# AleixMT/TrigenicInteractionPredictor

Measured on NVIDIA B200. Metric: EM link-updates/sec at K=10, higher is better.
Workload: dtype f64

## Files before the change

### include/tip.h

```cpp
#ifndef TIP_H_
#define TIP_H_

#include <stddef.h>
#include <stdint.h>

#ifdef __cplusplus
extern "C" {
#endif

#define TIP_ABI_VERSION 1
#define TIP_EPS 1e-10
#define TIP_R 2
#define TIP_MAX_K 32

#define TIP_EM_DEFAULT 0u
#define TIP_EM_FORCE_GENERIC 1u
#define TIP_EM_FP32_COMPUTE 2u
#define TIP_EM_GENE_SEGMENTED 8u
#define TIP_EM_SLOT_SEGMENTED 32u
#define TIP_EM_GATHER_L1 64u
#define TIP_EM_WITH_LOGLIK 4u

#define TIP_ROWS_COMPACT8 16u

// ... 13 lines not shown
int tip_order_rows_by_gene(const void *d_rows, int64_t n_rows, int64_t n_rows_r0, int P, void *d_ws, size_t ws_bytes,
                           void *d_rows_bc, void *stream);
int tip_order_rows(const void *d_rows, int64_t n_rows, int64_t n_rows_r0, void *d_ws, size_t ws_bytes, void *d_rows_bc,
                   void *stream);

int tip_em_workspace_bytes(int P, int K, int64_t n_rows, unsigned flags, size_t *bytes);
int tip_em_step(int P, int K, const void *d_rows, int64_t n_rows, int64_t n_rows_r0, const double *d_theta,
                const double *d_p, double *d_stats, void *d_ws, size_t ws_bytes, unsigned flags, void *stream);

int tip_em_step_host_rows(int P, int K, const void *h_rows, int64_t n_rows, int64_t n_rows_r0, unsigned row_flags,
                          void *d_rows_dev, const double *d_theta, const double *d_p, double *d_stats, void *d_ws,
                          size_t ws_bytes, unsigned *d_err, void *stream, void *copy_stream);

int tip_normalise(int P, int K, const double *d_stats, const int32_t *d_deg, double *d_theta, double *d_p,
                  void *stream);

size_t tip_loglik_workspace_bytes(int P, int K);
int tip_loglik(int P, int K, const void *d_rows, int64_t n_rows, int64_t n_rows_r0, const double *d_theta,
               const double *d_p, double *d_out, void *d_ws, unsigned flags, void *stream);

int tip_score(int P, int K, const int32_t *d_g1, const int32_t *d_g2, const int32_t *d_g3, int64_t T,
              const double *d_theta, const double *d_p, double *d_scores, void *stream);

int tip_metrics_workspace_bytes(int64_t T, size_t *bytes);
int tip_metrics(const double *d_scores, const int32_t *d_labels, int64_t T, int64_t positives_number,
                void *d_ws, size_t ws_bytes, int64_t *d_out, void *stream);

int tip_sort_scores_workspace_bytes(int64_t T, size_t *bytes);
int tip_sort_scores(const double *d_scores, int64_t T, void *d_ws, size_t ws_bytes, int32_t *d_order, double *d_sorted,
                    void *stream);
// ... 47 lines not shown
```

### trigenicinteractionpredictor_b200/_cabi.py

```python
from __future__ import annotations

import ctypes
import os
import re

HERE = os.path.dirname(os.path.abspath(__file__))
LIB_PATH = os.path.join(HERE, "libtip.so")
HEADER = os.path.join(os.path.dirname(HERE), "include", "tip.h")

c_void_p, c_int, c_int64, c_size_t, c_uint, c_double = (
    ctypes.c_void_p, ctypes.c_int, ctypes.c_int64, ctypes.c_size_t, ctypes.c_uint, ctypes.c_double)
_pi64 = ctypes.POINTER(ctypes.c_int64)
_psz = ctypes.POINTER(ctypes.c_size_t)
_pdbl = ctypes.POINTER(ctypes.c_double)

TIP_EM_DEFAULT = 0
TIP_EM_FORCE_GENERIC = 1
TIP_EM_FP32_COMPUTE = 2
TIP_EM_WITH_LOGLIK = 4
TIP_EM_GENE_SEGMENTED = 8
TIP_ROWS_COMPACT8 = 16
TIP_EM_SLOT_SEGMENTED = 32
TIP_EM_GATHER_L1 = 64

# ... 3 lines not shown
    "tip_stats_len": (c_int64, [c_int, c_int]),
    "tip_rows_capacity": (c_int64, [c_int64]),
    "tip_pack_rows_workspace_bytes": (c_int, [c_int64, _psz]),
    "tip_pack_rows": (c_int, [c_void_p, c_void_p, c_void_p, c_void_p, c_void_p, c_int64, c_int, c_void_p, c_size_t,
                              c_void_p, _pi64, _pi64, c_void_p, c_void_p]),
    "tip_order_rows_workspace_bytes": (c_int, [c_int64, _psz]),
    "tip_order_rows_out_bytes": (c_int64, [c_int64]),
    "tip_order_rows_by_gene": (c_int, [c_void_p, c_int64, c_int64, c_int, c_void_p, c_size_t, c_void_p, c_void_p]),
    "tip_order_rows": (c_int, [c_void_p, c_int64, c_int64, c_void_p, c_size_t, c_void_p, c_void_p]),
    "tip_em_workspace_bytes": (c_int, [c_int, c_int, c_int64, c_uint, _psz]),
    "tip_em_step": (c_int, [c_int, c_int, c_void_p, c_int64, c_int64, c_void_p, c_void_p, c_void_p, c_void_p, c_size_t,
                            c_uint, c_void_p]),
    "tip_em_step_host_rows": (c_int, [c_int, c_int, c_void_p, c_int64, c_int64, c_uint, c_void_p, c_void_p, c_void_p, c_void_p,
                                      c_void_p, c_size_t, c_void_p, c_void_p, c_void_p]),
    "tip_normalise": (c_int, [c_int, c_int, c_void_p, c_void_p, c_void_p, c_void_p, c_void_p]),
    "tip_loglik_workspace_bytes": (c_size_t, [c_int, c_int]),
    "tip_loglik": (c_int, [c_int, c_int, c_void_p, c_int64, c_int64, c_void_p, c_void_p, c_void_p, c_void_p, c_uint,
                           c_void_p]),
    "tip_score": (c_int, [c_int, c_int, c_void_p, c_void_p, c_void_p, c_int64, c_void_p, c_void_p, c_void_p, c_void_p]),
    "tip_metrics_workspace_bytes": (c_int, [c_int64, _psz]),
    "tip_metrics": (c_int, [c_void_p, c_void_p, c_int64, c_int64, c_void_p, c_size_t, c_void_p, c_void_p]),
    "tip_sort_scores_workspace_bytes": (c_int, [c_int64, _psz]),
    "tip_sort_scores": (c_int, [c_void_p, c_int64, c_void_p, c_size_t, c_void_p, c_void_p, c_void_p]),
    "tip_top_triplets_workspace_bytes": (c_int, [c_int, c_int, c_int, c_int64, c_int64, _psz]),
    "tip_top_triplets": (c_int, [c_int, c_int, c_int, c_void_p, c_void_p, c_void_p, c_int, c_void_p, c_int64, c_int64, c_void_p,
                                 c_size_t, c_void_p, c_void_p, _pi64, c_void_p]),
    "tip_top_triplets_last_passes": (c_int, []),
    "tip_reduce_samples": (c_int, [c_int, c_int64, c_void_p, c_void_p, c_void_p, c_void_p, c_void_p, c_void_p, c_void_p]),
    "tip_em_iterations_host": (c_int, [c_int, c_int, c_void_p, c_int64, c_int64, c_void_p, c_void_p, c_void_p, c_int,
                                       c_uint]),
# ... 81 lines not shown
```

### trigenicinteractionpredictor_b200/csrc/tip_api.cu

```cuda
#include <stdarg.h>
#include <string.h>

#include <chrono>

#include "tip_common.cuh"

namespace tip {

static thread_local char g_err[512] = "";

void set_error(const char *fmt, ...)
{
    va_list ap;
    va_start(ap, fmt);
    vsnprintf(g_err, sizeof(g_err), fmt, ap);
    va_end(ap);
}

static bool valid_K(int K) { return K >= 1 && K <= TIP_MAX_K; }
static bool uses_tuned(int K, unsigned flags)
{
    if (flags & TIP_EM_FORCE_GENERIC) return false;
    if (K <= 10) return true;
    return !(flags & (TIP_EM_WITH_LOGLIK | TIP_EM_FP32_COMPUTE));
// ... 10 lines not shown

extern "C" int64_t tip_stats_len(int P, int K) { return (int64_t)P * K + 2ll * K * K * K + 1; }

extern "C" int tip_em_workspace_bytes(int P, int K, int64_t n_rows, unsigned flags, size_t *bytes)
{
    TIP_REQUIRE(bytes != nullptr && P > 0 && valid_K(K) && n_rows >= 0, "tip_em_workspace_bytes: bad arguments");
    if (seg3_flag(flags)) {
        *bytes = em_seg3_workspace_bytes(P, K, n_rows);
        return 0;
    }
    *bytes = uses_tuned(K, flags) ? em_tuned_workspace_bytes(P, K, seg_flag(flags))
                                  : (size_t)(n_rows < 1 ? 1 : n_rows) * sizeof(double);
    return 0;
}

extern "C" int tip_em_step(int P, int K, const void *d_rows, int64_t n_rows, int64_t n_rows_r0, const double *d_theta,
                           const double *d_p, double *d_stats, void *d_ws, size_t ws_bytes, unsigned flags, void *stream)
{
    cudaStream_t st = reinterpret_cast<cudaStream_t>(stream);
    TIP_REQUIRE(P > 0 && valid_K(K), "tip_em_step: need P > 0 and 1 <= K <= %d (got P=%d K=%d)", TIP_MAX_K, P, K);
    TIP_REQUIRE(n_rows >= 0 && n_rows % 32 == 0 && n_rows_r0 >= 0 && n_rows_r0 <= n_rows && n_rows_r0 % 32 == 0,
                "tip_em_step: n_rows (%lld) and n_rows_r0 (%lld) must be multiples of 32 from tip_pack_rows",
                (long long)n_rows, (long long)n_rows_r0);
    TIP_REQUIRE(d_theta && d_p && d_stats && (d_rows || n_rows == 0), "tip_em_step: null pointer");
    TIP_REQUIRE(!(flags & TIP_EM_FP32_COMPUTE) || (K <= 10 && !(flags & (TIP_EM_FORCE_GENERIC | TIP_EM_WITH_LOGLIK))),
                "tip_em_step: TIP_EM_FP32_COMPUTE exists for the K <= 10 kernels only, without FORCE_GENERIC / WITH_LOGLIK");
    TIP_REQUIRE(!seg_flag(flags) || !(flags & (TIP_EM_FORCE_GENERIC | TIP_EM_WITH_LOGLIK | TIP_EM_FP32_COMPUTE)),
                "tip_em_step: TIP_EM_GENE_SEGMENTED cannot be combined with other mode flags");
    TIP_REQUIRE(!seg3_flag(flags) || (flags & ~(TIP_EM_SLOT_SEGMENTED | TIP_EM_GATHER_L1)) == 0,
                "tip_em_step: TIP_EM_SLOT_SEGMENTED combines with TIP_EM_GATHER_L1 only");
    TIP_REQUIRE(seg3_flag(flags) || !(flags & TIP_EM_GATHER_L1), "tip_em_step: TIP_EM_GATHER_L1 needs TIP_EM_SLOT_SEGMENTED");
    TIP_CHECK_CUDA(cudaMemsetAsync(d_stats, 0, sizeof(double) * (size_t)tip_stats_len(P, K), st));
    if (n_rows == 0) return 0;
    const int4 *rows = reinterpret_cast<const int4 *>(d_rows);
    if (seg3_flag(flags)) {
        const size_t need = em_seg3_workspace_bytes(P, K, n_rows);
        TIP_REQUIRE(d_ws != nullptr && ws_bytes >= need,
                    "tip_em_step: the slot-segmented mode needs %zu bytes of workspace (got %zu), see tip_em_workspace_bytes",
                    need, ws_bytes);
        return launch_em_seg3(P, K, rows, n_rows, n_rows_r0, d_theta, d_p, d_stats, reinterpret_cast<double *>(d_ws),
                              (flags & TIP_EM_GATHER_L1) != 0, st);
    }
    if (uses_tuned(K, flags)) {
        const size_t need = em_tuned_workspace_bytes(P, K, seg_flag(flags));
        TIP_REQUIRE(need == 0 || (d_ws != nullptr && ws_bytes >= need),
                    "tip_em_step: K=%d needs %zu bytes of workspace (got %zu), see tip_em_workspace_bytes", K, need, ws_bytes);
        bool handled = false;
        int rc = launch_em_tuned(P, K, rows, n_rows, n_rows_r0, d_theta, d_p, d_stats, reinterpret_cast<double *>(d_ws),
                                 (flags & TIP_EM_WITH_LOGLIK) != 0, (flags & TIP_EM_FP32_COMPUTE) != 0, seg_flag(flags), st,
                                 &handled);
        if (rc != 0 || handled) return rc;
    }
    TIP_REQUIRE(d_ws != nullptr && ws_bytes >= (size_t)n_rows * sizeof(double),
                "tip_em_step: the any-K path needs %zu bytes of workspace (got %zu)", (size_t)n_rows * sizeof(double), ws_bytes);
    return launch_em_generic(P, K, rows, n_rows, n_rows_r0, d_theta, d_p, d_stats, reinterpret_cast<double *>(d_ws), st);
}

extern "C" int tip_em_step_host_rows(int P, int K, const void *h_rows, int64_t n_rows, int64_t n_rows_r0, unsigned row_flags,
                                     void *d_rows_dev, const double *d_theta, const double *d_p, double *d_stats, void *d_ws,
                                     size_t ws_bytes, unsigned *d_err, void *stream, void *copy_stream)
{
    cudaStream_t st = reinterpret_cast<cudaStream_t>(stream), cs = reinterpret_cast<cudaStream_t>(copy_stream);
    TIP_REQUIRE(P > 0 && valid_K(K) && em_streamed_available(K, false, false, false),
                "tip_em_step_host_rows: the streamed E-step exists for the plain fp64 K <= 10 kernels (got K=%d); copy the "
                "rows and call tip_em_step", K);
    TIP_REQUIRE(n_rows > 0 && n_rows % 32 == 0 && n_rows_r0 >= 0 && n_rows_r0 <= n_rows && n_rows_r0 % 32 == 0,
                "tip_em_step_host_rows: n_rows (%lld) and n_rows_r0 (%lld) must be multiples of 32 from tip_pack_rows",
                (long long)n_rows, (long long)n_rows_r0);
    TIP_REQUIRE(h_rows && d_rows_dev && d_theta && d_p && d_stats && d_err && cs != st && (row_flags & ~TIP_ROWS_COMPACT8) == 0,
                "tip_em_step_host_rows: bad arguments (two distinct streams are required)");
// ... 172 lines not shown
        return rc;
    if (seg3 && n_iter > 0 && n_rows >= 32 && getenv("TIP_HOST_SEG3_AFTER_STREAM") == nullptr) {
        TIP_CHECK_CUDA(cudaMemcpyAsync(g.theta, h_theta, nth, cudaMemcpyHostToDevice, g.st));
        TIP_CHECK_CUDA(cudaMemcpyAsync(g.p, h_p, np, cudaMemcpyHostToDevice, g.st));
        TIP_CHECK_CUDA(cudaMemcpyAsync(compact ? g.rows8 : g.rows, h_rows, (size_t)n_rows * row_b, cudaMemcpyHostToDevice, g.st));
        if (compact && (rc = launch_rows_expand(g.rows8, g.rows, n_rows, g.st))) return rc;
        TIP_CHECK_CUDA(cudaEventRecord(g.ev_rows, g.st));
        TIP_CHECK_CUDA(cudaMemcpyAsync(g.deg, h_deg, (size_t)P * 4, cudaMemcpyHostToDevice, g.st));
        char *rows_bc = (char *)g.rows + (size_t)n_rows * 16;
        TIP_CHECK_CUDA(cudaStreamWaitEvent(g.copy, g.ev_rows, 0));
        if ((rc = order_rows_parts(g.rows, n_rows, n_rows_r0, g.order_ws2, g.order_ws2_b, rows_bc, g.copy, 2, P))) return rc;
        TIP_CHECK_CUDA(cudaEventRecord(g.ev_ordered, g.copy));
        if ((rc = order_rows_parts(g.rows, n_rows, n_rows_r0, g.order_ws, g.order_ws_b, rows_bc, g.st, 1, P))) return rc;
        for (int it = 0; it < n_iter; ++it) {
            if (it == 0) seg3_wait_before_bc(g.ev_ordered);
            rc = tip_em_step(P, K, g.rows, n_rows, n_rows_r0, (const double *)g.theta, (const double *)g.p, (double *)g.stats,
                             g.ws, g.ws_b, flags, g.st);
            if (rc) return rc;
            rc = launch_normalise(P, K, (const double *)g.stats, (const int32_t *)g.deg, (double *)g.theta, (double *)g.p, g.st);
            if (rc) return rc;
        }
        TIP_CHECK_CUDA(cudaMemcpyAsync(h_theta, g.theta, nth, cudaMemcpyDeviceToHost, g.st));
        TIP_CHECK_CUDA(cudaMemcpyAsync(h_p, g.p, np, cudaMemcpyDeviceToHost, g.st));
        TIP_CHECK_CUDA(cudaStreamSynchronize(g.st));
        return 0;
    }
    const bool tuned = uses_tuned(K, flags & ~(TIP_EM_SLOT_SEGMENTED | TIP_EM_GATHER_L1));
    const bool streamed = tuned && n_iter > 0 && n_rows >= 32 * kHostChunks &&
                          em_streamed_available(K, (flags & TIP_EM_WITH_LOGLIK) != 0, (flags & TIP_EM_FP32_COMPUTE) != 0,
                                                seg_flag(flags)) && getenv("TIP_HOST_NO_STREAM") == nullptr;
    char *s_dst = compact ? (char *)g.rows8 : (char *)g.rows;
    TIP_CHECK_CUDA(cudaMemcpyAsync(g.theta, h_theta, nth, cudaMemcpyHostToDevice, g.st));
    TIP_CHECK_CUDA(cudaMemcpyAsync(g.p, h_p, np, cudaMemcpyHostToDevice, g.st));
    if (!streamed) TIP_CHECK_CUDA(cudaMemcpyAsync(g.deg, h_deg, (size_t)P * 4, cudaMemcpyHostToDevice, g.st));
// ... 288 lines not shown
```

### trigenicinteractionpredictor_b200/csrc/tip_common.cuh

```cuda
#pragma once
#include <cuda_runtime.h>
#include <stdint.h>
#include <stdio.h>

#include "tip.h"

namespace tip {

constexpr int kWarp = 32;
constexpr int kNumSM_B200 = 148;

void set_error(const char *fmt, ...);

#define TIP_CHECK_CUDA(expr)                                                                   \
    do {                                                                                       \
        cudaError_t _e = (expr);                                                               \
        if (_e != cudaSuccess) {                                                               \
            ::tip::set_error("%s failed: %s (%s:%d)", #expr, cudaGetErrorString(_e), __FILE__, \
                             __LINE__);                                                        \
            return -2;                                                                         \
        }                                                                                      \
    } while (0)

#define TIP_REQUIRE(cond, ...)             \
// ... 44 lines not shown
template <int N>
__device__ __forceinline__ void cp_async_wait()
{
    asm volatile("cp.async.wait_group %0;" ::"n"(N) : "memory");
}

__host__ __device__ inline int64_t stats_off_S(int P, int K) { return (int64_t)P * K; }
__host__ __device__ inline int64_t stats_off_ll(int P, int K) { return (int64_t)P * K + 2ll * K * K * K; }

int launch_em_generic(int P, int K, const int4 *rows, int64_t n_rows, int64_t n_rows_r0, const double *theta,
                      const double *p, double *stats, double *s_ws, cudaStream_t st);
int launch_em_tuned(int P, int K, const int4 *rows, int64_t n_rows, int64_t n_rows_r0, const double *theta,
                    const double *p, double *stats, double *ws, bool with_ll, bool f32, bool seg, cudaStream_t st,
                    bool *handled, int phases = 7);
size_t em_tuned_workspace_bytes(int P, int K, bool seg);
int launch_em_seg3(int P, int K, const int4 *rows, int64_t n_rows, int64_t n_rows_r0, const double *theta, const double *p,
                   double *stats, double *ws, bool gather_l1, cudaStream_t st);
size_t em_seg3_workspace_bytes(int P, int K, int64_t n_rows);
int order_rows_parts(const void *d_rows, int64_t n_rows, int64_t n_rows_r0, void *d_ws, size_t ws_bytes, void *d_rows_bc,
                     cudaStream_t st, int parts, int P);
void seg3_wait_before_bc(cudaEvent_t ev);
cudaEvent_t seg3_take_bc_wait();
bool em_streamed_available(int K, bool with_ll, bool f32, bool seg);
int launch_em_streamed(int P, int K, const void *rows, int64_t n_rows, int64_t n_rows_r0, const double *theta, double *stats,
                       double *ws, unsigned *err, unsigned long long *chk, bool compact, cudaStream_t st);
int launch_stream_verify(const void *rows, int64_t n_rows, bool compact, unsigned long long *chk, unsigned *err, cudaStream_t st);
int launch_loglik(int P, int K, const int4 *rows, int64_t n_rows, int64_t n_rows_r0, const double *theta, const double *p,
                  double *out, void *ws, bool force_generic, cudaStream_t st);
int launch_loglik_seg(int P, int K, const int4 *rows, int64_t n_rows, const double *theta, const double *p, double *out,
                      double *partials, unsigned *counter, int max_blocks, double *Zws, cudaStream_t st);
size_t loglik_seg_workspace_bytes(int P, int K);
int launch_loglik_tuned(int K, const int4 *rows, int64_t n_rows, int64_t n_rows_r0, const double *theta, const double *p,
// ... 9 lines not shown
```

### trigenicinteractionpredictor_b200/csrc/tip_seg3.cu

```cuda
#include <stdlib.h>

#include <cub/device/device_radix_sort.cuh>

#include "tip_common.cuh"

namespace tip {

__device__ __forceinline__ void dmma884(double &c0, double &c1, double a, double b)
{
    asm volatile("mma.sync.aligned.m8n8k4.row.col.f64.f64.f64.f64 {%0,%1}, {%2}, {%3}, {%0,%1};"
                 : "+d"(c0), "+d"(c1)
                 : "d"(a), "d"(b));
}

__device__ __forceinline__ void red_add_f64_nz3(double *addr, double v)
{
    asm volatile("{ .reg .pred p; setp.neu.f64 p, %1, 0d0000000000000000; @p red.global.add.f64 [%0], %1; }" ::"l"(addr),
                 "d"(v)
                 : "memory");
}

__device__ __forceinline__ void st_relaxed_gpu_f64(double *addr, double v)
{
    asm volatile("st.relaxed.gpu.global.f64 [%0], %1;" ::"l"(addr), "d"(v) : "memory");
// ... 93 lines not shown
            copy(idw[l * 4 + 1 + slot], l, slot, (rem - slot * C::U) * C::UNIT);
        }
    }
}

template <int K, bool FIRST, int NST, bool CA>
__global__ void __launch_bounds__(32, K <= 16 ? (FIRST ? 16 : 18) : 1) seg3_pass_kernel(const S3Args a)
{
    using C = S3<K>;
    constexpr int KK = C::KK, NB = C::NB, NKG = C::NKG, RS = C::RS, D = NST - 1;
    extern __shared__ __align__(16) unsigned char smem_raw[];
    const int lane = threadIdx.x, li = lane & 3, ri = lane >> 2;
    if constexpr (FIRST) {
        asm volatile("griddepcontrol.wait;" ::: "memory");
        asm volatile("griddepcontrol.launch_dependents;" ::: "memory");
    }
    auto stage_of = [&](int b) { return reinterpret_cast<double *>(smem_raw + (size_t)b * C::BUF_BYTES); };
    auto ids_of = [&](int b) { return reinterpret_cast<int4 *>(stage_of(b) + 32 * RS + 32); };
    int xo[NB];
    bool xv[NB];
#pragma unroll
    for (int i = 0; i < NB; ++i) {
        xv[i] = i * 8 + ri < K;
        xo[i] = xv[i] ? i * 8 + ri : 0;
    }

    double acc[NB][NB][2];
#pragma unroll
    for (int i = 0; i < NB; ++i)
#pragma unroll
// ... 276 lines not shown
        __syncwarp();
#pragma unroll
        for (int j = 0; j + 1 < D + RQ; ++j) tq[j] = tq[j + 1];
        tq[D + RQ - 1] = tn;
        if (++cb == NST) cb = 0;
    }
}

constexpr int kPrepGenes = 16;
__global__ void __launch_bounds__(256) seg3_prep_kernel(int P, int K, const double *__restrict__ theta,
                                                        const double *__restrict__ p, double *__restrict__ Zg,
                                                        double *__restrict__ PT, double *__restrict__ thpad, int TP,
                                                        double2 *__restrict__ zero2, int64_t n_zero2,
                                                        double2 *__restrict__ nan2, int64_t n_nan2,
                                                        unsigned *__restrict__ cnt_a, unsigned cnt_a0,
                                                        unsigned *__restrict__ cnt_bc, unsigned cnt_bc0)
{
    asm volatile("griddepcontrol.launch_dependents;" ::: "memory");
    if (blockIdx.x == 0 && threadIdx.x == 0) {
        *cnt_a = cnt_a0;
        *cnt_bc = cnt_bc0;
    }
    extern __shared__ double psm[];
    const int KK = K * K, K3 = KK * K;
    const bool staged = K <= 20;
    double *tsm = psm + (staged ? 2 * K3 : 0);
    const int g0 = blockIdx.x * kPrepGenes;
    const int ng = (P - g0 < kPrepGenes) ? P - g0 : kPrepGenes;
    constexpr int PB = 8;
    double pv[PB];
    const int e_th = threadIdx.x;
    double tv = 0.0;
    if (e_th < ng * K) tv = __ldg(theta + (int64_t)g0 * K + e_th);
    if (staged) {
#pragma unroll
        for (int j = 0; j < PB; ++j) {
            const int e = threadIdx.x + j * 256;
// ... 54 lines not shown
        else if (slot == 1) { i = x; j = k; l = y; }
        else { i = x; j = y; l = k; }
        PT[f] = __ldg(p + (((int64_t)i * K + j) * K + l) * 2 + r);
    }
}

constexpr int kFin3Threads = 96;
constexpr int kFin3GeneChunk = 96;
constexpr int kS3MaxPeers = 16;

struct S3Push {
    int n;
    double *dst[kS3MaxPeers];
};

template <int K>
__global__ void __launch_bounds__(kFin3Threads) seg3_finish_kernel(int P, const double *__restrict__ theta,
                                                                     const double *__restrict__ PT,
                                                                     const double *__restrict__ Mg, double *__restrict__ stats,
                                                                     const S3Push push)
{
    constexpr int KK = K * K, K3 = KK * K, NB = (K + 7) / 8, NBC = (KK + 7) / 8;
    const int lane = threadIdx.x & 31, li = lane & 3, ri = lane >> 2, warp = threadIdx.x >> 5;
    const int n_groups = (P + 7) / 8;
    const int n_chunks = (P + kFin3GeneChunk - 1) / kFin3GeneChunk, n_kind2 = 2 * NBC * n_chunks;
    __shared__ double csm[2][NB * 2][32];
    if ((int)blockIdx.x < n_groups) {
        const int slot = warp, g = blockIdx.x * 8 + ri;
        const bool gv = g < P;
        double c[NB][2];
#pragma unroll
        for (int i = 0; i < NB; ++i) c[i][0] = c[i][1] = 0.0;
        constexpr int NE = (KK + 3) / 4;
        constexpr int EB = NE < 32 ? NE : 32;
        for (int r = 0; r < 2; ++r) {
            const double *Mrow = Mg + ((int64_t)(slot * 2 + r) * P + (gv ? g : 0)) * KK;
// ... 24 lines not shown
            for (int i = 0; i < NB; ++i) {
                csm[warp - 1][2 * i][lane] = c[i][0];
                csm[warp - 1][2 * i + 1][lane] = c[i][1];
            }
        }
        __syncthreads();
        if (warp == 0) {
            __shared__ __align__(16) double rowbuf[8 * K + 2];
            if (gv) {
#pragma unroll
                for (int i = 0; i < NB; ++i)
#pragma unroll
                    for (int h = 0; h < 2; ++h) {
                        const int k = i * 8 + 2 * li + h;
                        if (k < K)
                            rowbuf[ri * K + k] = __ldg(theta + (int64_t)g * K + k) *
                                                 ((c[i][h] + csm[0][2 * i + h][lane]) + csm[1][2 * i + h][lane]);
                    }
            }
            __syncwarp();
            const int g0 = blockIdx.x * 8, ng = (P - g0 < 8) ? P - g0 : 8, nd = ng * K;
            const int64_t at0 = (int64_t)g0 * K;
            for (int q = -1; q < push.n; ++q) {
                double *dst = (q < 0 ? stats : push.dst[q]) + at0;
                for (int i = lane; i < nd / 2; i += 32) reinterpret_cast<double2 *>(dst)[i] = reinterpret_cast<const double2 *>(rowbuf)[i];
                if ((nd & 1) && lane == 0) dst[nd - 1] = rowbuf[nd - 1];
            }
        }
        return;
    }
    const int wt = ((int)blockIdx.x - n_groups) * (kFin3Threads / 32) + warp;
    if (wt < n_kind2) {
        const int w2 = wt;
        const int chunk = w2 / (2 * NBC), rem = w2 - chunk * (2 * NBC), r = rem / NBC, bcb = rem - r * NBC;
        const int g_lo = chunk * kFin3GeneChunk, g_hi = (g_lo + kFin3GeneChunk < P) ? g_lo + kFin3GeneChunk : P;
        const int bc = bcb * 8 + ri;
        const double *Mr = Mg + (int64_t)r * P * KK;
        double c[NB][2];
#pragma unroll
        for (int i = 0; i < NB; ++i) c[i][0] = c[i][1] = 0.0;
#pragma unroll 4
        for (int g0 = g_lo; g0 < g_hi; g0 += 4) {
            const int g = g0 + li;
            const bool gv = g < g_hi;
            const double bv = (gv && bc < KK) ? __ldg(Mr + (int64_t)g * KK + bc) : 0.0;
#pragma unroll
            for (int i = 0; i < NB; ++i) {
                const int al = i * 8 + ri;
                const double av = (gv && al < K) ? __ldg(theta + (int64_t)g * K + al) : 0.0;
                dmma884(c[i][0], c[i][1], av, bv);
            }
        }
        double *S = stats + stats_off_S(P, K) + (int64_t)r * K3;
#pragma unroll
        for (int i = 0; i < NB; ++i)
#pragma unroll
            for (int h = 0; h < 2; ++h) {
                const int al = i * 8 + ri, cell = bcb * 8 + 2 * li + h;
                if (al < K && cell < KK) red_add_f64_nz3(S + (int64_t)al * KK + cell, c[i][h]);
            }
    }
}

struct S3Layout {
    size_t off_M, off_cnt, off_Z, off_PT, off_T, off_s, total;
};
static S3Layout s3_layout(int P, int K, int64_t n_rows)
{
    const size_t KK = (size_t)K * K;
    S3Layout l;
    l.off_M = 0;
    l.off_cnt = 6 * (size_t)P * KK;
    l.off_Z = l.off_cnt + kS3CounterDoubles;
    l.off_PT = l.off_Z + 2 * (size_t)P * KK;
    l.off_PT = (l.off_PT + 1) / 2 * 2;
// ... 45 lines not shown
    if (!g_s3_ev[0])
        for (int j = 0; j < 6; ++j) TIP_CHECK_CUDA(cudaEventCreate(&g_s3_ev[j]));
    TIP_CHECK_CUDA(cudaEventRecord(g_s3_ev[i], st));
    return 0;
}

static bool s3_no_overlap()
{
    static int v = -1;
    if (v < 0) {
        const char *e = getenv("TIP_SEG3_NO_OVERLAP");
        v = (e && atoi(e) != 0) ? 1 : 0;
    }
    return v != 0;
}

template <int K, bool FIRST, int NST, bool CA>
static int s3_launch_pass_n(const S3Args &a, cudaStream_t st, int *grid_only)
{
    using C = S3<K>;
    constexpr size_t smem = C::BUF_BYTES * NST;
    static int blocks_per_sm = 0;
    if (blocks_per_sm == 0) {
        TIP_CHECK_CUDA(cudaFuncSetAttribute(seg3_pass_kernel<K, FIRST, NST, CA>, cudaFuncAttributeMaxDynamicSharedMemorySize, (int)smem));
        TIP_CHECK_CUDA(cudaFuncSetAttribute(seg3_pass_kernel<K, FIRST, NST, CA>, cudaFuncAttributePreferredSharedMemoryCarveout,
                                            cudaSharedmemCarveoutMaxShared));
        int nb = 0;
        TIP_CHECK_CUDA(cudaOccupancyMaxActiveBlocksPerMultiprocessor(&nb, seg3_pass_kernel<K, FIRST, NST, CA>, 32, smem));
        TIP_REQUIRE(nb >= 1, "seg3_pass_kernel<%d> does not fit on an SM (smem %zu)", K, smem);
        blocks_per_sm = nb;
// ... 25 lines not shown
}

template <int K, bool FIRST>
static int s3_launch_pass(const S3Args &a, cudaStream_t st, int *grid_only = nullptr)
{
    const bool ca = (a.tune & 1) != 0;
    if (s3_stages(FIRST) == 1)
        return ca ? s3_launch_pass_n<K, FIRST, 1, true>(a, st, grid_only) : s3_launch_pass_n<K, FIRST, 1, false>(a, st, grid_only);
    return ca ? s3_launch_pass_n<K, FIRST, 2, true>(a, st, grid_only) : s3_launch_pass_n<K, FIRST, 2, false>(a, st, grid_only);
}

static S3Push g_s3_push = {};

template <int K>
static int launch_em_seg3_k(int P, const int4 *rows, int64_t n_rows, int64_t n_rows_r0, const double *theta, const double *p,
                            double *stats, double *ws, bool gather_l1, cudaStream_t st)
{
    const S3Push push = g_s3_push;
    g_s3_push.n = 0;
    const cudaEvent_t bc_wait = seg3_take_bc_wait();
    const S3Layout l = s3_layout(P, K, n_rows);
    const int KK = K * K;
    TIP_REQUIRE(n_rows / 32 < (1ll << 27), "tip_em_step: too many tiles in one shard for the slot-segmented kernels");
    const int skip = s3_skip();
    S3Args a;
    a.P = P;
    a.rows = rows;
    a.tiles_per_order = (int)(n_rows / 32);
    a.n_tiles_r0 = (int)(n_rows_r0 / 32);
    a.theta = ws + l.off_T;
    a.Zg = ws + l.off_Z;
// ... 6 lines not shown
    const int *sched = reinterpret_cast<const int *>(rows + 3 * n_rows);
    a.sched = sched;
    a.n_sched = a.tiles_per_order;
    S3Args bc = a;
    bc.rows = rows + n_rows;
    bc.n_tiles = 2 * a.tiles_per_order;
    bc.slot0 = 1;
    bc.counter = reinterpret_cast<unsigned *>(ws + l.off_cnt) + kS3Groups * 32;
    bc.sched = sched + a.tiles_per_order;
    bc.n_sched = 2 * a.tiles_per_order;
    int grid_a = 0, grid_bc = 0;
    int rc = s3_launch_pass<K, true>(a, st, &grid_a);
    if (rc) return rc;
    rc = s3_launch_pass<K, false>(bc, st, &grid_bc);
    if (rc) return rc;
    if (s3_mark(0, st)) return -2;
    if (s3_mark(1, st)) return -2;
    {
        const size_t smem = sizeof(double) * ((K <= 20 ? 2 * KK * K : 0) + kPrepGenes * K);
        static bool attr = false;
        if (!attr && smem > 48 * 1024) {
            TIP_CHECK_CUDA(cudaFuncSetAttribute(seg3_prep_kernel, cudaFuncAttributeMaxDynamicSharedMemorySize, 128 * 1024));
            attr = true;
        }
        seg3_prep_kernel<<<(P + kPrepGenes - 1) / kPrepGenes, 256, smem, st>>>(
            P, K, theta, p, ws + l.off_Z, ws + l.off_PT, ws + l.off_T, S3<K>::TP, reinterpret_cast<double2 *>(ws + l.off_M),
            (int64_t)l.off_cnt / 2, reinterpret_cast<double2 *>(ws + l.off_s), (n_rows < 32 ? 32 : n_rows) / 2, a.counter,
            2u * (unsigned)grid_a, bc.counter, 2u * (unsigned)grid_bc);
        TIP_CHECK_CUDA(cudaGetLastError());
    }
    if (s3_mark(2, st)) return -2;
    rc = (skip & 4) ? 0 : s3_launch_pass<K, true>(a, st);
    if (rc) return rc;
    if (s3_mark(3, st)) return -2;
    if (bc_wait) {
        TIP_CHECK_CUDA(cudaStreamWaitEvent(st, bc_wait, 0));
        bc.tune |= 16;
    }
    rc = (skip & 8) ? 0 : s3_launch_pass<K, false>(bc, st);
    if (rc) return rc;
    if (s3_mark(4, st)) return -2;
    if (!(skip & 16)) {
        constexpr int NBC = (K * K + 7) / 8;
        const int n_kind2 = 2 * NBC * ((P + kFin3GeneChunk - 1) / kFin3GeneChunk);
        const int wpc = kFin3Threads / 32;
        seg3_finish_kernel<K><<<(P + 7) / 8 + (n_kind2 + wpc - 1) / wpc, kFin3Threads, 0, st>>>(P, theta, ws + l.off_PT, ws + l.off_M,
                                                                                             stats, push);
        TIP_CHECK_CUDA(cudaGetLastError());
    }
    if (s3_mark(5, st)) return -2;
    return 0;
}

int launch_em_seg3(int P, int K, const int4 *rows, int64_t n_rows, int64_t n_rows_r0, const double *theta, const double *p,
                   double *stats, double *ws, bool gather_l1, cudaStream_t st)
{
    switch (K) {
#define TIP_S3_CASE(k) \
    case k: return launch_em_seg3_k<k>(P, rows, n_rows, n_rows_r0, theta, p, stats, ws, gather_l1, st);
        TIP_S3_CASE(1) TIP_S3_CASE(2) TIP_S3_CASE(3) TIP_S3_CASE(4) TIP_S3_CASE(5) TIP_S3_CASE(6) TIP_S3_CASE(7) TIP_S3_CASE(8)
        TIP_S3_CASE(9) TIP_S3_CASE(10) TIP_S3_CASE(11) TIP_S3_CASE(12) TIP_S3_CASE(13) TIP_S3_CASE(14) TIP_S3_CASE(15)
        TIP_S3_CASE(16) TIP_S3_CASE(17) TIP_S3_CASE(18) TIP_S3_CASE(19) TIP_S3_CASE(20) TIP_S3_CASE(21) TIP_S3_CASE(22)
        TIP_S3_CASE(23) TIP_S3_CASE(24) TIP_S3_CASE(25) TIP_S3_CASE(26) TIP_S3_CASE(27) TIP_S3_CASE(28) TIP_S3_CASE(29)
        TIP_S3_CASE(30) TIP_S3_CASE(31) TIP_S3_CASE(32)
#undef TIP_S3_CASE
        default: set_error("launch_em_seg3: K = %d out of range", K); return -1;
    }
}

constexpr unsigned kOrderPadBit = 1u << 20, kOrderRatingShift = 21;

__global__ void order_keys_kernel(const int4 *__restrict__ rows, int64_t n_rows, int64_t n_rows_r0, int slot,
                                  unsigned *__restrict__ keys, int32_t *__restrict__ vals)
{
// ... 285 lines not shown
```

### trigenicinteractionpredictor_b200/engine.py

```python
from __future__ import annotations

import ctypes
import functools
import os

import numpy as np
import torch

from . import _cabi
from . import dist as _dist

_PROCESS_DEVICE = None


def _ptr(t):
    return ctypes.c_void_p(t.data_ptr()) if t is not None else ctypes.c_void_p(0)


def _on_device(fn):
    @functools.wraps(fn)
    def wrapper(self, *args, **kwargs):
        with torch.cuda.device(self.device):
            return fn(self, *args, **kwargs)
    return wrapper


class PackedLinks:

    def __init__(self, rows, n_rows, n_rows_r0, n_real, deg):
        self.rows, self.n_rows, self.n_rows_r0, self.n_real, self.deg = rows, n_rows, n_rows_r0, n_real, deg
        self.rows3 = None
        self.rows3_buf = None
        self.order_ws = None


def default_flags(K: int) -> int:
    return _cabi.TIP_EM_SLOT_SEGMENTED if K >= 4 else _cabi.TIP_EM_DEFAULT


class EMEngine:
    def __init__(self, P: int, K: int, device=None, group=None, flags: int | None = None,
                 exchange: str = "peer"):
        if not torch.cuda.is_available():
            raise _cabi.TipLibraryError("no CUDA device: trigenicinteractionpredictor_b200 has no CPU path")
        self.lib = _cabi.load()
        self.P, self.K = int(P), int(K)
        self.device = torch.device(device if device is not None else "cuda:%d" % torch.cuda.current_device())
        if self.device.index is None:
# ... 193 lines not shown
        _cabi.check(self.lib.tip_peer_barrier(self.peer.flag_ptrs, _ptr(self.peer.epoch), self.peer.rank,
                                              self.peer.world, self._stream()), "tip_peer_barrier")
        _cabi.check(self.lib.tip_normalise_peers(self.P, self.K, self.peer.stats_ptrs[par], self.peer.world,
                                                 _ptr(self.train.deg), _ptr(self.theta), _ptr(self.p),
                                                 self._stream()), "tip_normalise_peers")
        self.launches += 2

    @_on_device
    def em_step(self, stats=None):
        t = self.train
        stats = self.stats if stats is None else stats
        seg3 = bool(self.flags & _cabi.TIP_EM_SLOT_SEGMENTED)
        _cabi.check(self.lib.tip_em_step(self.P, self.K, _ptr(t.rows3 if seg3 else t.rows), t.n_rows, t.n_rows_r0, _ptr(self.theta),
                                         _ptr(self.p), _ptr(stats), _ptr(self.em_ws), self.em_ws_bytes,
                                         self.flags, self._stream()), "tip_em_step")
        if self.flags & _cabi.TIP_EM_SLOT_SEGMENTED:
            self.launches += 4
        else:
            self.launches += 3 if (self.K > 4 and not (self.flags & _cabi.TIP_EM_FORCE_GENERIC)) else 2

    @_on_device
    def em_step_host_rows(self, h_rows: torch.Tensor, compact: bool, stats=None):
        t = self.train
        stats = self.stats if stats is None else stats
        if getattr(self, "_copy_stream", None) is None:
            self._copy_stream = torch.cuda.Stream(self.device)
            self._stream_err = torch.zeros(64, dtype=torch.int32, device=self.device)
            self._rows_dev = None
        need = t.n_rows * (8 if compact else 16)
        if self._rows_dev is None or self._rows_dev.numel() < need:
            self._rows_dev = torch.empty(need, dtype=torch.uint8, device=self.device)
        _cabi.check(self.lib.tip_em_step_host_rows(
            self.P, self.K, ctypes.c_void_p(h_rows.data_ptr()), t.n_rows, t.n_rows_r0,
            _cabi.TIP_ROWS_COMPACT8 if compact else 0, _ptr(self._rows_dev), _ptr(self.theta), _ptr(self.p), _ptr(stats),
# ... 28 lines not shown
        self.launches += 1

    @_on_device
    def _iteration_body(self, par):
        if self.peer is not None:
            if self.peer.mode == "rs":
                par = 0
            fused = (self.peer.mode == "push" and bool(self.flags & _cabi.TIP_EM_SLOT_SEGMENTED) and self.train.n_rows > 0
                     and os.environ.get("TIP_PEER_FUSED", "1") != "0")
            if fused:
                pe = self.peer
                _cabi.check(self.lib.tip_em_set_push_targets(pe.inbox_ptrs[par], pe.rank, pe.world, pe.n_pad),
                            "tip_em_set_push_targets")
            self.em_step(self.peer.stats(par))
            self._peer_mstep(par, theta_pushed=fused)
            return
        self.em_step()
        if self.pairs is not None:
            self._pairs_estep(self.stats)
        if self.world > 1:
            _dist.allreduce_sum_(self.stats, self.group)
        self.normalise()
        if self.pairs is not None:
            self._pairs_mstep()

    def em_iteration(self):
        self._iteration_body(self._iter & 1)
        self._iter += 1

    @_on_device
# ... 126 lines not shown
```

Before: 6.100 billion.

## Fuse M-step normalisation into seg3 finish kernel with PDL launch

Adds tip_em_iteration, which on the slot-segmented path folds the M-step into the finish kernel. Theta is normalised per gene inside the finish kernel, and the last block (tracked by an atomic counter) normalises p. The stats memset moves into the prep kernel, and the finish kernel is launched with programmatic stream serialization so it can overlap the previous kernel's tail. This removes the separate memset and normalise launches, at the cost of a last-block-done serial tail and extra complexity in the finish kernel.

```diff
diff --git a/include/tip.h b/include/tip.h
--- a/include/tip.h
+++ b/include/tip.h
@@ -51,6 +51,9 @@
 
 int tip_normalise(int P, int K, const double *d_stats, const int32_t *d_deg, double *d_theta, double *d_p,
                   void *stream);
+
+int tip_em_iteration(int P, int K, const void *d_rows, int64_t n_rows, int64_t n_rows_r0, double *d_theta, double *d_p,
+                     double *d_stats, void *d_ws, size_t ws_bytes, unsigned flags, const int32_t *d_deg, void *stream);
 
 size_t tip_loglik_workspace_bytes(int P, int K);
 int tip_loglik(int P, int K, const void *d_rows, int64_t n_rows, int64_t n_rows_r0, const double *d_theta,
diff --git a/trigenicinteractionpredictor_b200/_cabi.py b/trigenicinteractionpredictor_b200/_cabi.py
--- a/trigenicinteractionpredictor_b200/_cabi.py
+++ b/trigenicinteractionpredictor_b200/_cabi.py
@@ -41,6 +41,8 @@
     "tip_em_step_host_rows": (c_int, [c_int, c_int, c_void_p, c_int64, c_int64, c_uint, c_void_p, c_void_p, c_void_p, c_void_p,
                                       c_void_p, c_size_t, c_void_p, c_void_p, c_void_p]),
     "tip_normalise": (c_int, [c_int, c_int, c_void_p, c_void_p, c_void_p, c_void_p, c_void_p]),
+    "tip_em_iteration": (c_int, [c_int, c_int, c_void_p, c_int64, c_int64, c_void_p, c_void_p, c_void_p, c_void_p, c_size_t,
+                                 c_uint, c_void_p, c_void_p]),
     "tip_loglik_workspace_bytes": (c_size_t, [c_int, c_int]),
     "tip_loglik": (c_int, [c_int, c_int, c_void_p, c_int64, c_int64, c_void_p, c_void_p, c_void_p, c_void_p, c_uint,
                            c_void_p]),
diff --git a/trigenicinteractionpredictor_b200/csrc/tip_api.cu b/trigenicinteractionpredictor_b200/csrc/tip_api.cu
--- a/trigenicinteractionpredictor_b200/csrc/tip_api.cu
+++ b/trigenicinteractionpredictor_b200/csrc/tip_api.cu
@@ -48,10 +48,9 @@
     return 0;
 }
 
-extern "C" int tip_em_step(int P, int K, const void *d_rows, int64_t n_rows, int64_t n_rows_r0, const double *d_theta,
-                           const double *d_p, double *d_stats, void *d_ws, size_t ws_bytes, unsigned flags, void *stream)
-{
-    cudaStream_t st = reinterpret_cast<cudaStream_t>(stream);
+static int em_step(int P, int K, const void *d_rows, int64_t n_rows, int64_t n_rows_r0, const double *d_theta, const double *d_p,
+                   double *d_stats, void *d_ws, size_t ws_bytes, unsigned flags, cudaStream_t st, const S3MStep &ms)
+{
     TIP_REQUIRE(P > 0 && valid_K(K), "tip_em_step: need P > 0 and 1 <= K <= %d (got P=%d K=%d)", TIP_MAX_K, P, K);
     TIP_REQUIRE(n_rows >= 0 && n_rows % 32 == 0 && n_rows_r0 >= 0 && n_rows_r0 <= n_rows && n_rows_r0 % 32 == 0,
                 "tip_em_step: n_rows (%lld) and n_rows_r0 (%lld) must be multiples of 32 from tip_pack_rows",
@@ -64,7 +63,8 @@
     TIP_REQUIRE(!seg3_flag(flags) || (flags & ~(TIP_EM_SLOT_SEGMENTED | TIP_EM_GATHER_L1)) == 0,
                 "tip_em_step: TIP_EM_SLOT_SEGMENTED combines with TIP_EM_GATHER_L1 only");
     TIP_REQUIRE(seg3_flag(flags) || !(flags & TIP_EM_GATHER_L1), "tip_em_step: TIP_EM_GATHER_L1 needs TIP_EM_SLOT_SEGMENTED");
-    TIP_CHECK_CUDA(cudaMemsetAsync(d_stats, 0, sizeof(double) * (size_t)tip_stats_len(P, K), st));
+    if (!(seg3_flag(flags) && n_rows > 0 && seg3_fused()))
+        TIP_CHECK_CUDA(cudaMemsetAsync(d_stats, 0, sizeof(double) * (size_t)tip_stats_len(P, K), st));
     if (n_rows == 0) return 0;
     const int4 *rows = reinterpret_cast<const int4 *>(d_rows);
     if (seg3_flag(flags)) {
@@ -73,7 +73,7 @@
                     "tip_em_step: the slot-segmented mode needs %zu bytes of workspace (got %zu), see tip_em_workspace_bytes",
                     need, ws_bytes);
         return launch_em_seg3(P, K, rows, n_rows, n_rows_r0, d_theta, d_p, d_stats, reinterpret_cast<double *>(d_ws),
-                              (flags & TIP_EM_GATHER_L1) != 0, st);
+                              (flags & TIP_EM_GATHER_L1) != 0, st, ms);
     }
     if (uses_tuned(K, flags)) {
         const size_t need = em_tuned_workspace_bytes(P, K, seg_flag(flags));
@@ -88,6 +88,30 @@
     TIP_REQUIRE(d_ws != nullptr && ws_bytes >= (size_t)n_rows * sizeof(double),
                 "tip_em_step: the any-K path needs %zu bytes of workspace (got %zu)", (size_t)n_rows * sizeof(double), ws_bytes);
     return launch_em_generic(P, K, rows, n_rows, n_rows_r0, d_theta, d_p, d_stats, reinterpret_cast<double *>(d_ws), st);
+}
+
+extern "C" int tip_em_step(int P, int K, const void *d_rows, int64_t n_rows, int64_t n_rows_r0, const double *d_theta,
+                           const double *d_p, double *d_stats, void *d_ws, size_t ws_bytes, unsigned flags, void *stream)
+{
+    return em_step(P, K, d_rows, n_rows, n_rows_r0, d_theta, d_p, d_stats, d_ws, ws_bytes, flags,
+                   reinterpret_cast<cudaStream_t>(stream), S3MStep{});
+}
+
+extern "C" int tip_em_iteration(int P, int K, const void *d_rows, int64_t n_rows, int64_t n_rows_r0, double *d_theta, double *d_p,
+                                double *d_stats, void *d_ws, size_t ws_bytes, unsigned flags, const int32_t *d_deg, void *stream)
+{
+    cudaStream_t st = reinterpret_cast<cudaStream_t>(stream);
+    TIP_REQUIRE(d_deg != nullptr, "tip_em_iteration: null d_deg");
+    if (seg3_flag(flags) && n_rows > 0 && seg3_fused()) {
+        S3MStep ms;
+        ms.deg = d_deg;
+        ms.theta = d_theta;
+        ms.p = d_p;
+        return em_step(P, K, d_rows, n_rows, n_rows_r0, d_theta, d_p, d_stats, d_ws, ws_bytes, flags, st, ms);
+    }
+    const int rc = em_step(P, K, d_rows, n_rows, n_rows_r0, d_theta, d_p, d_stats, d_ws, ws_bytes, flags, st, S3MStep{});
+    if (rc) return rc;
+    return tip_normalise(P, K, d_stats, d_deg, d_theta, d_p, stream);
 }
 
 extern "C" int tip_em_step_host_rows(int P, int K, const void *h_rows, int64_t n_rows, int64_t n_rows_r0, unsigned row_flags,
@@ -290,10 +314,8 @@
         if ((rc = order_rows_parts(g.rows, n_rows, n_rows_r0, g.order_ws, g.order_ws_b, rows_bc, g.st, 1, P))) return rc;
         for (int it = 0; it < n_iter; ++it) {
             if (it == 0) seg3_wait_before_bc(g.ev_ordered);
-            rc = tip_em_step(P, K, g.rows, n_rows, n_rows_r0, (const double *)g.theta, (const double *)g.p, (double *)g.stats,
-                             g.ws, g.ws_b, flags, g.st);
-            if (rc) return rc;
-            rc = launch_normalise(P, K, (const double *)g.stats, (const int32_t *)g.deg, (double *)g.theta, (double *)g.p, g.st);
+            rc = tip_em_iteration(P, K, g.rows, n_rows, n_rows_r0, (double *)g.theta, (double *)g.p, (double *)g.stats, g.ws,
+                                  g.ws_b, flags, (const int32_t *)g.deg, g.st);
             if (rc) return rc;
         }
         TIP_CHECK_CUDA(cudaMemcpyAsync(h_theta, g.theta, nth, cudaMemcpyDeviceToHost, g.st));
diff --git a/trigenicinteractionpredictor_b200/csrc/tip_common.cuh b/trigenicinteractionpredictor_b200/csrc/tip_common.cuh
--- a/trigenicinteractionpredictor_b200/csrc/tip_common.cuh
+++ b/trigenicinteractionpredictor_b200/csrc/tip_common.cuh
@@ -82,8 +82,13 @@
                     const double *p, double *stats, double *ws, bool with_ll, bool f32, bool seg, cudaStream_t st,
                     bool *handled, int phases = 7);
 size_t em_tuned_workspace_bytes(int P, int K, bool seg);
+struct S3MStep {
+    const int32_t *deg = nullptr;
+    double *theta = nullptr, *p = nullptr;
+};
 int launch_em_seg3(int P, int K, const int4 *rows, int64_t n_rows, int64_t n_rows_r0, const double *theta, const double *p,
-                   double *stats, double *ws, bool gather_l1, cudaStream_t st);
+                   double *stats, double *ws, bool gather_l1, cudaStream_t st, const S3MStep &ms);
+bool seg3_fused();
 size_t em_seg3_workspace_bytes(int P, int K, int64_t n_rows);
 int order_rows_parts(const void *d_rows, int64_t n_rows, int64_t n_rows_r0, void *d_ws, size_t ws_bytes, void *d_rows_bc,
                      cudaStream_t st, int parts, int P);
diff --git a/trigenicinteractionpredictor_b200/csrc/tip_seg3.cu b/trigenicinteractionpredictor_b200/csrc/tip_seg3.cu
--- a/trigenicinteractionpredictor_b200/csrc/tip_seg3.cu
+++ b/trigenicinteractionpredictor_b200/csrc/tip_seg3.cu
@@ -131,6 +131,8 @@
     if constexpr (FIRST) {
         asm volatile("griddepcontrol.wait;" ::: "memory");
         asm volatile("griddepcontrol.launch_dependents;" ::: "memory");
+    } else {
+        asm volatile("griddepcontrol.launch_dependents;" ::: "memory");
     }
     auto stage_of = [&](int b) { return reinterpret_cast<double *>(smem_raw + (size_t)b * C::BUF_BYTES); };
     auto ids_of = [&](int b) { return reinterpret_cast<int4 *>(stage_of(b) + 32 * RS + 32); };
@@ -437,13 +439,16 @@
                                                         double2 *__restrict__ zero2, int64_t n_zero2,
                                                         double2 *__restrict__ nan2, int64_t n_nan2,
                                                         unsigned *__restrict__ cnt_a, unsigned cnt_a0,
-                                                        unsigned *__restrict__ cnt_bc, unsigned cnt_bc0)
+                                                        unsigned *__restrict__ cnt_bc, unsigned cnt_bc0,
+                                                        unsigned *__restrict__ cnt_s, double *__restrict__ zero_s, int n_zero_s)
 {
     asm volatile("griddepcontrol.launch_dependents;" ::: "memory");
     if (blockIdx.x == 0 && threadIdx.x == 0) {
         *cnt_a = cnt_a0;
         *cnt_bc = cnt_bc0;
-    }
+        *cnt_s = 0u;
+    }
+    for (int i = blockIdx.x * blockDim.x + threadIdx.x; i < n_zero_s; i += gridDim.x * blockDim.x) zero_s[i] = 0.0;
     extern __shared__ double psm[];
     const int KK = K * K, K3 = KK * K;
     const bool staged = K <= 20;
@@ -528,12 +533,20 @@
     double *dst[kS3MaxPeers];
 };
 
+struct S3FinMStep {
+    const int32_t *deg;
+    double *theta;
+    double *p;
+    unsigned *s_done;
+};
+
 template <int K>
-__global__ void __launch_bounds__(kFin3Threads) seg3_finish_kernel(int P, const double *__restrict__ theta,
+__global__ void __launch_bounds__(kFin3Threads) seg3_finish_kernel(int P, const double *__restrict__ theta, int TP,
                                                                      const double *__restrict__ PT,
                                                                      const double *__restrict__ Mg, double *__restrict__ stats,
-                                                                     const S3Push push)
-{
+                                                                     const S3Push push, const S3FinMStep ms)
+{
+    asm volatile("griddepcontrol.wait;" ::: "memory");
     constexpr int KK = K * K, K3 = KK * K, NB = (K + 7) / 8, NBC = (KK + 7) / 8;
     const int lane = threadIdx.x & 31, li = lane & 3, ri = lane >> 2, warp = threadIdx.x >> 5;
     const int n_groups = (P + 7) / 8;
@@ -588,7 +601,7 @@
                     for (int h = 0; h < 2; ++h) {
                         const int k = i * 8 + 2 * li + h;
                         if (k < K)
-                            rowbuf[ri * K + k] = __ldg(theta + (int64_t)g * K + k) *
+                            rowbuf[ri * K + k] = __ldg(theta + (int64_t)g * TP + k) *
                                                  ((c[i][h] + csm[0][2 * i + h][lane]) + csm[1][2 * i + h][lane]);
                     }
             }
@@ -600,6 +613,8 @@
                 for (int i = lane; i < nd / 2; i += 32) reinterpret_cast<double2 *>(dst)[i] = reinterpret_cast<const double2 *>(rowbuf)[i];
                 if ((nd & 1) && lane == 0) dst[nd - 1] = rowbuf[nd - 1];
             }
+            if (ms.deg != nullptr)
+                for (int i = lane; i < nd; i += 32) ms.theta[at0 + i] = rowbuf[i] / (double)__ldg(ms.deg + g0 + i / K);
         }
         return;
     }
@@ -621,7 +636,7 @@
 #pragma unroll
             for (int i = 0; i < NB; ++i) {
                 const int al = i * 8 + ri;
-                const double av = (gv && al < K) ? __ldg(theta + (int64_t)g * K + al) : 0.0;
+                const double av = (gv && al < K) ? __ldg(theta + (int64_t)g * TP + al) : 0.0;
                 dmma884(c[i][0], c[i][1], av, bv);
             }
         }
@@ -633,6 +648,27 @@
                 const int al = i * 8 + ri, cell = bcb * 8 + 2 * li + h;
                 if (al < K && cell < KK) red_add_f64_nz3(S + (int64_t)al * KK + cell, c[i][h]);
             }
+        if (ms.deg != nullptr) {
+            __threadfence();
+            __syncwarp();
+            unsigned prev = 0;
+            if (lane == 0) prev = atomicAdd(ms.s_done, 1u);
+            prev = __shfl_sync(0xffffffffu, prev, 0);
+            if (prev == (unsigned)n_kind2 - 1u) {
+                __threadfence();
+                const double *Sa = stats + stats_off_S(P, K);
+#pragma unroll 4
+                for (int cell = lane; cell < K3; cell += 32) {
+                    const double n0 = ms.p[2 * cell] * __ldcg(Sa + cell);
+                    const double n1 = ms.p[2 * cell + 1] * __ldcg(Sa + K3 + cell);
+                    double d = TIP_EPS;
+                    d += n0;
+                    d += n1;
+                    ms.p[2 * cell] = n0 / d;
+                    ms.p[2 * cell + 1] = n1 / d;
+                }
+            }
+        }
     }
 }
 
@@ -708,6 +744,17 @@
     }
     return v != 0;
 }
+
+static bool s3_fused_env()
+{
+    static int v = -1;
+    if (v < 0) {
+        const char *e = getenv("TIP_SEG3_FUSED");
+        v = (e && atoi(e) == 0) ? 0 : 1;
+    }
+    return v != 0;
+}
+bool seg3_fused() { return s3_fused_env() && !g_s3_timing && s3_skip() == 0; }
 
 template <int K, bool FIRST, int NST, bool CA>
 static int s3_launch_pass_n(const S3Args &a, cudaStream_t st, int *grid_only)
@@ -763,7 +810,7 @@
 
 template <int K>
 static int launch_em_seg3_k(int P, const int4 *rows, int64_t n_rows, int64_t n_rows_r0, const double *theta, const double *p,
-                            double *stats, double *ws, bool gather_l1, cudaStream_t st)
+                            double *stats, double *ws, bool gather_l1, cudaStream_t st, const S3MStep &mstep)
 {
     const S3Push push = g_s3_push;
     g_s3_push.n = 0;
@@ -800,6 +847,9 @@
     if (rc) return rc;
     rc = s3_launch_pass<K, false>(bc, st, &grid_bc);
     if (rc) return rc;
+    const bool fused = seg3_fused();
+    TIP_REQUIRE(fused || mstep.deg == nullptr, "launch_em_seg3: the M-step is fused only in the fused launch sequence");
+    unsigned *cnt_s = a.counter + 32;
     if (s3_mark(0, st)) return -2;
     if (s3_mark(1, st)) return -2;
     {
@@ -812,7 +862,8 @@
         seg3_prep_kernel<<<(P + kPrepGenes - 1) / kPrepGenes, 256, smem, st>>>(
             P, K, theta, p, ws + l.off_Z, ws + l.off_PT, ws + l.off_T, S3<K>::TP, reinterpret_cast<double2 *>(ws + l.off_M),
             (int64_t)l.off_cnt / 2, reinterpret_cast<double2 *>(ws + l.off_s), (n_rows < 32 ? 32 : n_rows) / 2, a.counter,
-            2u * (unsigned)grid_a, bc.counter, 2u * (unsigned)grid_bc);
+            2u * (unsigned)grid_a, bc.counter, 2u * (unsigned)grid_bc, cnt_s, fused ? stats + stats_off_S(P, K) : nullptr,
+            fused ? 2 * KK * K + 1 : 0);
         TIP_CHECK_CUDA(cudaGetLastError());
     }
     if (s3_mark(2, st)) return -2;
@@ -830,20 +881,29 @@
         constexpr int NBC = (K * K + 7) / 8;
         const int n_kind2 = 2 * NBC * ((P + kFin3GeneChunk - 1) / kFin3GeneChunk);
         const int wpc = kFin3Threads / 32;
-        seg3_finish_kernel<K><<<(P + 7) / 8 + (n_kind2 + wpc - 1) / wpc, kFin3Threads, 0, st>>>(P, theta, ws + l.off_PT, ws + l.off_M,
-                                                                                             stats, push);
-        TIP_CHECK_CUDA(cudaGetLastError());
+        const S3FinMStep ms = {mstep.deg, mstep.theta, mstep.p, cnt_s};
+        cudaLaunchConfig_t cfg = {};
+        cfg.gridDim = dim3((P + 7) / 8 + (n_kind2 + wpc - 1) / wpc);
+        cfg.blockDim = dim3(kFin3Threads);
+        cfg.stream = st;
+        cudaLaunchAttribute attr[1];
+        attr[0].id = cudaLaunchAttributeProgrammaticStreamSerialization;
+        attr[0].val.programmaticStreamSerializationAllowed = 1;
+        cfg.attrs = attr;
+        cfg.numAttrs = fused ? 1 : 0;
+        TIP_CHECK_CUDA(cudaLaunchKernelEx(&cfg, seg3_finish_kernel<K>, P, (const double *)(ws + l.off_T), (int)S3<K>::TP,
+                                          (const double *)(ws + l.off_PT), (const double *)(ws + l.off_M), stats, push, ms));
     }
     if (s3_mark(5, st)) return -2;
     return 0;
 }
 
 int launch_em_seg3(int P, int K, const int4 *rows, int64_t n_rows, int64_t n_rows_r0, const double *theta, const double *p,
-                   double *stats, double *ws, bool gather_l1, cudaStream_t st)
+                   double *stats, double *ws, bool gather_l1, cudaStream_t st, const S3MStep &mstep)
 {
     switch (K) {
 #define TIP_S3_CASE(k) \
-    case k: return launch_em_seg3_k<k>(P, rows, n_rows, n_rows_r0, theta, p, stats, ws, gather_l1, st);
+    case k: return launch_em_seg3_k<k>(P, rows, n_rows, n_rows_r0, theta, p, stats, ws, gather_l1, st, mstep);
         TIP_S3_CASE(1) TIP_S3_CASE(2) TIP_S3_CASE(3) TIP_S3_CASE(4) TIP_S3_CASE(5) TIP_S3_CASE(6) TIP_S3_CASE(7) TIP_S3_CASE(8)
         TIP_S3_CASE(9) TIP_S3_CASE(10) TIP_S3_CASE(11) TIP_S3_CASE(12) TIP_S3_CASE(13) TIP_S3_CASE(14) TIP_S3_CASE(15)
         TIP_S3_CASE(16) TIP_S3_CASE(17) TIP_S3_CASE(18) TIP_S3_CASE(19) TIP_S3_CASE(20) TIP_S3_CASE(21) TIP_S3_CASE(22)
diff --git a/trigenicinteractionpredictor_b200/engine.py b/trigenicinteractionpredictor_b200/engine.py
--- a/trigenicinteractionpredictor_b200/engine.py
+++ b/trigenicinteractionpredictor_b200/engine.py
@@ -32,6 +32,10 @@
         self.rows3 = None
         self.rows3_buf = None
         self.order_ws = None
+
+
+def _seg3_fused() -> bool:
+    return os.environ.get("TIP_SEG3_FUSED", "1") != "0" and int(os.environ.get("TIP_SEG3_SKIP", "0") or 0) == 0
 
 
 def default_flags(K: int) -> int:
@@ -255,10 +259,22 @@
         _cabi.check(self.lib.tip_em_step(self.P, self.K, _ptr(t.rows3 if seg3 else t.rows), t.n_rows, t.n_rows_r0, _ptr(self.theta),
                                          _ptr(self.p), _ptr(stats), _ptr(self.em_ws), self.em_ws_bytes,
                                          self.flags, self._stream()), "tip_em_step")
+        self.launches += self._em_step_launches()
+
+    def _em_step_launches(self):
         if self.flags & _cabi.TIP_EM_SLOT_SEGMENTED:
-            self.launches += 4
-        else:
-            self.launches += 3 if (self.K > 4 and not (self.flags & _cabi.TIP_EM_FORCE_GENERIC)) else 2
+            return 4
+        return 3 if (self.K > 4 and not (self.flags & _cabi.TIP_EM_FORCE_GENERIC)) else 2
+
+    @_on_device
+    def em_iteration_single(self):
+        t = self.train
+        seg3 = bool(self.flags & _cabi.TIP_EM_SLOT_SEGMENTED)
+        _cabi.check(self.lib.tip_em_iteration(self.P, self.K, _ptr(t.rows3 if seg3 else t.rows), t.n_rows,
+                                              t.n_rows_r0, _ptr(self.theta), _ptr(self.p), _ptr(self.stats), _ptr(self.em_ws),
+                                              self.em_ws_bytes, self.flags, _ptr(t.deg), self._stream()), "tip_em_iteration")
+        fused_mstep = seg3 and t.n_rows > 0 and _seg3_fused()
+        self.launches += self._em_step_launches() + (0 if fused_mstep else 1)
 
     @_on_device
     def em_step_host_rows(self, h_rows: torch.Tensor, compact: bool, stats=None):
@@ -317,6 +333,9 @@
                             "tip_em_set_push_targets")
             self.em_step(self.peer.stats(par))
             self._peer_mstep(par, theta_pushed=fused)
+            return
+        if self.pairs is None and self.world == 1:
+            self.em_iteration_single()
             return
         self.em_step()
         if self.pairs is not None:
```

Result: slower. 4.693 billion, median of 6 (-23.1%).
